# C-bowman/inference-tools

Hardware: AMD Instinct MI355X
Metric: GpRegressor fit+predict wall-time and GFLOP/s at N=16384, d=8; % fp64 MFMA peak (higher is better)
Workload: dtype f64

## Files before the change

inference-tools_amd/csrc/gemm_tiles.h:

```cpp
#pragma once
#include "gpmi_internal.h"

#ifndef GPMI_C_PLAIN
#define GPMI_C_LOAD(p) __builtin_nontemporal_load(p)
#define GPMI_C_STORE(v, p) __builtin_nontemporal_store(v, p)
#else
#define GPMI_C_LOAD(p) (*(p))
#define GPMI_C_STORE(v, p) (*(p) = (v))
#endif

namespace gemm_tiles {

constexpr int CST_NT = 0, CST_SC1 = 1;
template <int CST>
__device__ __forceinline__ void c_store_begin() {
  if (CST == CST_SC1) asm volatile("s_nop 15\n\ts_nop 15" ::: "memory");
}
template <int CST>
__device__ __forceinline__ void c_store(d2_t v, d2_t* p) {
  if (CST == CST_SC1)
    asm volatile("global_store_dwordx4 %0, %1, off sc1\n\ts_nop 1" ::"v"(p), "v"(v) : "memory");
  else
    GPMI_C_STORE(v, p);
}
template <int CST>
__device__ __forceinline__ void c_store(double v, double* p) {
  if (CST == CST_SC1)
    asm volatile("global_store_dwordx2 %0, %1, off sc1" ::"v"(p), "v"(v) : "memory");
  else
    GPMI_C_STORE(v, p);
}

constexpr int BK = 16;
constexpr int LDS_STRIDE = 18;
#ifndef GPMI_SMALL_PF
#define GPMI_SMALL_PF 4
#endif

template <int BKN, int BM, int BN>
constexpr int staged_lds_doubles() {
  return 2 * (BM * LDS_STRIDE + (BKN ? BK * (BN + 16) : BN * LDS_STRIDE));
}

template <int OP, int BKN, int BM, int BN, int CST = CST_NT, bool BTRI = false>
__device__ __forceinline__ void staged_tile(const double* __restrict__ Ag, const double* __restrict__ Bg, double* Cg,
                                            int64_t lda, int64_t ldb, int64_t ldc, int nk, double* smem) {
  static_assert(!BTRI || (BKN == 0 && BN == 128 && OP == OP_ASSIGN), "BTRI: the in-place panel TRSM only");
  constexpr int CSTEP = BTRI ? 32 : 16;
  constexpr int TM = BM / 32, TN = BN / 32;
  constexpr int LDS_STRIDE_KN = BN + 16;
  constexpr int A_DOUBLES = BM * LDS_STRIDE;
  constexpr int B_DOUBLES = BKN ? BK * LDS_STRIDE_KN : BN * LDS_STRIDE;
  constexpr int BUF_DOUBLES = A_DOUBLES + B_DOUBLES;
  const int tid = threadIdx.x;
  const int lane = tid & 63, wave = tid >> 6;
  const int wr = wave >> 1, wc = wave & 1;

  const int lrow = tid >> 3, lkc = (tid & 7) * 2;
  const int lkc_sw = lkc ^ ((((lrow & 15) >= 4) && ((lrow & 15) < 12)) ? 4 : 0);
  const int nrow = tid / (BN / 2), nnc = (tid % (BN / 2)) * 2;
  constexpr int PF = (BM * BN < 128 * 128) ? GPMI_SMALL_PF : 1;
  d2_t ra[PF][TM], rb[PF][TN];
  unsigned voa[TM], vob[TN];
#pragma unroll
  for (int i = 0; i < TM; ++i) voa[i] = (unsigned)(((int64_t)(lrow + 32 * i) * lda + lkc) * 8);
#pragma unroll
  for (int i = 0; i < TN; ++i)
    vob[i] = BKN ? (unsigned)(((int64_t)(nrow + (512 / BN) * i) * ldb + nnc) * 8)
                 : (unsigned)(((int64_t)(lrow + 32 * i) * ldb + lkc) * 8);
  auto gload = [&](int k0, int slot) {
    const char* ab = reinterpret_cast<const char*>(Ag + k0);
    const char* bb = reinterpret_cast<const char*>(BKN ? Bg + (int64_t)k0 * ldb : Bg + k0);
#pragma unroll
    for (int i = 0; i < TM; ++i) ra[slot][i] = *reinterpret_cast<const d2_t*>(ab + voa[i]);
#pragma unroll
    for (int i = 0; i < TN; ++i) rb[slot][i] = *reinterpret_cast<const d2_t*>(bb + vob[i]);
  };
  auto sstore = [&](int buf, int slot) {
    double* sa = smem + buf * BUF_DOUBLES;
    double* sb = sa + A_DOUBLES;
#pragma unroll
    for (int i = 0; i < TM; ++i)
      *reinterpret_cast<d2_t*>(sa + (lrow + 32 * i) * LDS_STRIDE + lkc_sw) = (OP == OP_SUB) ? -ra[slot][i] : ra[slot][i];
#pragma unroll
    for (int i = 0; i < TN; ++i) {
      if (BKN)
        *reinterpret_cast<d2_t*>(sb + (nrow + (512 / BN) * i) * LDS_STRIDE_KN + nnc) = rb[slot][i];
      else
        *reinterpret_cast<d2_t*>(sb + (lrow + 32 * i) * LDS_STRIDE + lkc_sw) = rb[slot][i];
    }
  };

  const int fr = lane & 15, fk = lane >> 4;
  const int wcol = BTRI ? wc * 16 : wc * (BN / 2);
  Cg += (int64_t)(wr * (BM / 2)) * ldc + wcol;
  const int sw = (fr >= 4 && fr < 12) ? 1 : 0;
  const int a_off = (wr * (BM / 2) + fr) * LDS_STRIDE + ((fk ^ sw) << 2);
  const int b_off = BKN ? 4 * fk * LDS_STRIDE_KN + wc * (BN / 2) + fr
                        : (wcol + fr) * LDS_STRIDE + ((fk ^ sw) << 2);

  const int klast = (nk - 1) * BK;
  auto gload_clamped = [&](int kt, int slot) { gload(kt < nk ? kt * BK : klast, slot); };
  if (PF == 1) gload(0, 0);
  d4_t acc[TM][TN];
#pragma unroll
  for (int i = 0; i < TM; ++i)
#pragma unroll
    for (int j = 0; j < TN; ++j) {
      if (OP == OP_SUB) {
#pragma unroll
        for (int r = 0; r < 4; ++r) acc[i][j][r] = GPMI_C_LOAD(&Cg[(int64_t)(i * 16 + fk + 4 * r) * ldc + j * CSTEP + fr]);
      } else {
        acc[i][j] = d4_t{0.0, 0.0, 0.0, 0.0};
      }
    }
  if (PF > 1) {
    gload(0, 0);
#pragma unroll
    for (int p = 1; p < PF; ++p) gload_clamped(p, p);
  }
  sstore(0, 0);
  __syncthreads();
  auto kstep = [&](int kt, int slot_free, int slot_next) {
    const int cur = kt & 1;
    if (PF == 1) {
      if (kt + 1 < nk) gload((kt + 1) * BK, 0);
    } else {
      gload_clamped(kt + PF, slot_free);
    }
    const double* sa = smem + cur * BUF_DOUBLES;
    const double* sb = sa + A_DOUBLES;
#pragma unroll
    for (int h = 0; h < 2; ++h) {
      d2_t a[TM], b[TN];
#pragma unroll
      for (int t = 0; t < TM; ++t)
        a[t] = *reinterpret_cast<const d2_t*>(sa + a_off + t * 16 * LDS_STRIDE + 2 * h);
#pragma unroll
      for (int t = 0; t < TN; ++t) {
        if (BKN)
          b[t] = d2_t{sb[b_off + (2 * h) * LDS_STRIDE_KN + t * 16],
                      sb[b_off + (2 * h + 1) * LDS_STRIDE_KN + t * 16]};
        else
          b[t] = *reinterpret_cast<const d2_t*>(sb + b_off + t * CSTEP * LDS_STRIDE + 2 * h);
      }
#pragma unroll
      for (int j = 0; j < TN; ++j) {
        if (BTRI && kt > 2 * j + wc) continue;
#pragma unroll
        for (int q = 0; q < 2; ++q)
#pragma unroll
          for (int i = 0; i < TM; ++i)
            acc[i][j] = __builtin_amdgcn_mfma_f64_16x16x4f64(a[i][q], b[j][q], acc[i][j], 0, 0, 0);
      }
    }
    if (PF > 1 || kt + 1 < nk) sstore(cur ^ 1, slot_next);
    __syncthreads();
  };
  if (PF == 1) {
    kstep(0, 0, 0);
    for (int kt = 1; kt < nk; ++kt) kstep(kt, 0, 0);
  } else {
    for (int kb = 0; kb < nk; kb += PF) {
#pragma unroll
      for (int u = 0; u < PF; ++u) {
        if (kb + u >= nk) break;
        kstep(kb + u, u, (1 + u) % PF);
      }
    }
  }

  c_store_begin<CST>();
#pragma unroll
  for (int i = 0; i < TM; ++i)
#pragma unroll
    for (int j = 0; j < TN; ++j)
#pragma unroll
      for (int r = 0; r < 4; ++r) c_store<CST>(acc[i][j][r], &Cg[(int64_t)(i * 16 + fk + 4 * r) * ldc + j * CSTEP + fr]);
}

constexpr int DMA_BK = 8;
#ifndef GPMI_DMA_STAGES
#define GPMI_DMA_STAGES 4
#endif
constexpr int DMA_STAGES = GPMI_DMA_STAGES;
constexpr int DMA_OP_DOUBLES = 128 * DMA_BK;
constexpr int DMA128_LDS_DOUBLES = DMA_STAGES * 2 * DMA_OP_DOUBLES;
constexpr int DMA64_LDS_DOUBLES = DMA_STAGES * 2 * 64 * DMA_BK;

__device__ inline void dma_wait(int newer) {
  if (newer >= 12) asm volatile("s_waitcnt vmcnt(12)" ::: "memory");
  else if (newer >= 8) asm volatile("s_waitcnt vmcnt(8)" ::: "memory");
  else if (newer >= 4) asm volatile("s_waitcnt vmcnt(4)" ::: "memory");
  else asm volatile("s_waitcnt vmcnt(0)" ::: "memory");
}

template <int OP, int CST = CST_NT>
__device__ __forceinline__ void dma128_tile(const double* __restrict__ Ag, const double* __restrict__ Bg, double* Cg,
                                            int64_t lda, int64_t ldb, int64_t ldc, int nk, double* smem) {
  const int tid = threadIdx.x, lane = tid & 63, wave = tid >> 6;
  const int wr = wave >> 1, wc = wave & 1;
  const int fr = lane & 15, fk = lane >> 4;
  const int row0 = tid >> 2, slot = tid & 3;
  const int q0 = (slot - 2 * ((row0 >> 2) & 3)) & 3;
  const double* a_src0 = Ag + (int64_t)row0 * lda + 2 * q0;
  const double* a_src1 = a_src0 + (int64_t)64 * lda;
  auto bperm = [](int R) {
    const int t = (R >> 4) & 3, f = R & 15;
    return (R & 64) + ((t & 2) << 4) + 2 * f + (t & 1);
  };
  const double* b_src0 = Bg + (int64_t)bperm(row0) * ldb + 2 * q0;
  const double* b_src1 = Bg + (int64_t)bperm(row0 + 64) * ldb + 2 * q0;
  const unsigned lds0 = (unsigned)(uintptr_t)smem;
  const unsigned wave_off = (unsigned)__builtin_amdgcn_readfirstlane(wave * 64 * 16);
  auto issue = [&](int st, int k0) {
    const unsigned base = lds0 + (unsigned)st * (2 * DMA_OP_DOUBLES * 8) + wave_off;
    const double* p0 = a_src0 + k0;
    const double* p1 = a_src1 + k0;
    const double* p2 = b_src0 + k0;
    const double* p3 = b_src1 + k0;
    asm volatile(
        "s_mov_b32 m0, %4\n\ts_nop 0\n\tglobal_load_lds_dwordx4 %0, off\n\t"
        "s_mov_b32 m0, %5\n\ts_nop 0\n\tglobal_load_lds_dwordx4 %1, off\n\t"
        "s_mov_b32 m0, %6\n\ts_nop 0\n\tglobal_load_lds_dwordx4 %2, off\n\t"
        "s_mov_b32 m0, %7\n\ts_nop 0\n\tglobal_load_lds_dwordx4 %3, off"
        :
        : "v"(p0), "v"(p1), "v"(p2), "v"(p3), "s"(base), "s"(base + 256 * 16), "s"(base + DMA_OP_DOUBLES * 8),
          "s"(base + DMA_OP_DOUBLES * 8 + 256 * 16)
        : "memory");
  };
  for (int st = 0; st < DMA_STAGES - 1 && st < nk; ++st) issue(st, st * DMA_BK);

  Cg += (int64_t)(wr * 64) * ldc + wc * 64;
  d4_t acc[4][4];
#pragma unroll
  for (int i = 0; i < 4; ++i)
#pragma unroll
    for (int jp = 0; jp < 2; ++jp)
#pragma unroll
      for (int r = 0; r < 4; ++r) {
        d2_t cv = d2_t{0.0, 0.0};
        if (OP == OP_SUB)
          cv = GPMI_C_LOAD(reinterpret_cast<const d2_t*>(&Cg[(int64_t)(i * 16 + fk + 4 * r) * ldc + jp * 32 + 2 * fr]));
        acc[i][2 * jp][r] = cv[0];
        acc[i][2 * jp + 1][r] = cv[1];
      }

  const int rslot = (fk + 2 * (fr >> 2)) & 3;
  const int a_off = ((wr * 64 + fr) * 4 + rslot) * 2;
  const int b_off = DMA_OP_DOUBLES + ((wc * 64 + fr) * 4 + rslot) * 2;
  auto stage = [&](int kt) {
    const int ahead = nk - 1 - kt;
    dma_wait(4 * (ahead < DMA_STAGES - 2 ? ahead : DMA_STAGES - 2));
    __syncthreads();
#ifdef GPMI_DMA_ISSUE_EARLY
    if (kt + DMA_STAGES - 1 < nk) issue((kt + DMA_STAGES - 1) % DMA_STAGES, (kt + DMA_STAGES - 1) * DMA_BK);
#endif
    const double* sa = smem + (kt % DMA_STAGES) * 2 * DMA_OP_DOUBLES;
    d2_t a[4], b[4];
#pragma unroll
    for (int t = 0; t < 4; ++t) {
      a[t] = *reinterpret_cast<const d2_t*>(sa + a_off + t * 16 * 4 * 2);
    }
#pragma unroll
    for (int t = 0; t < 4; ++t) b[t] = *reinterpret_cast<const d2_t*>(sa + b_off + t * 16 * 4 * 2);
#ifndef GPMI_DMA_ISSUE_EARLY
    if (kt + DMA_STAGES - 1 < nk) issue((kt + DMA_STAGES - 1) % DMA_STAGES, (kt + DMA_STAGES - 1) * DMA_BK);
#endif
#pragma unroll
    for (int h = 0; h < 2; ++h)
#pragma unroll
      for (int i = 0; i < 4; ++i)
#pragma unroll
        for (int j = 0; j < 4; ++j)
          acc[i][j] = __builtin_amdgcn_mfma_f64_16x16x4f64(a[i][h], b[j][h], acc[i][j], 0, 0, OP == OP_SUB ? 1 : 0);
  };
  stage(0);
  int kt = 1;
  for (; kt + 3 < nk; kt += 4) {
    stage(kt);
    stage(kt + 1);
    stage(kt + 2);
    stage(kt + 3);
  }
  for (; kt < nk; ++kt) stage(kt);
  c_store_begin<CST>();
#pragma unroll
  for (int i = 0; i < 4; ++i)
#pragma unroll
    for (int jp = 0; jp < 2; ++jp)
#pragma unroll
      for (int r = 0; r < 4; ++r)
        c_store<CST>((d2_t{acc[i][2 * jp][r], acc[i][2 * jp + 1][r]}),
                     reinterpret_cast<d2_t*>(&Cg[(int64_t)(i * 16 + fk + 4 * r) * ldc + jp * 32 + 2 * fr]));
}

template <int OP, int CST = CST_NT>
__device__ __forceinline__ void dma64_tile(const double* __restrict__ Ag, const double* __restrict__ Bg, double* Cg,
                                           int64_t lda, int64_t ldb, int64_t ldc, int nk, double* smem) {
  constexpr int OPD = 64 * DMA_BK;
  const int tid = threadIdx.x, lane = tid & 63, wave = tid >> 6;
  const int wr = wave >> 1, wc = wave & 1;
  const int fr = lane & 15, fk = lane >> 4;
  const int row0 = tid >> 2, slot = tid & 3;
  const int q0 = (slot - 2 * ((row0 >> 2) & 3)) & 3;
  const double* a_src = Ag + (int64_t)row0 * lda + 2 * q0;
  const int bcol = (row0 & 32) + 2 * (row0 & 15) + ((row0 >> 4) & 1);
  const double* b_src = Bg + (int64_t)bcol * ldb + 2 * q0;
  const unsigned lds0 = (unsigned)(uintptr_t)smem;
  const unsigned wave_off = (unsigned)__builtin_amdgcn_readfirstlane(wave * 64 * 16);
  auto issue = [&](int st, int k0) {
    const unsigned base = lds0 + (unsigned)st * (2 * OPD * 8) + wave_off;
    const double* p0 = a_src + k0;
    const double* p1 = b_src + k0;
    asm volatile(
        "s_mov_b32 m0, %2\n\ts_nop 0\n\tglobal_load_lds_dwordx4 %0, off\n\t"
        "s_mov_b32 m0, %3\n\ts_nop 0\n\tglobal_load_lds_dwordx4 %1, off"
        :
        : "v"(p0), "v"(p1), "s"(base), "s"(base + OPD * 8)
        : "memory");
  };
  for (int st = 0; st < DMA_STAGES - 1 && st < nk; ++st) issue(st, st * DMA_BK);

  Cg += (int64_t)(wr * 32) * ldc + wc * 32;
  d4_t acc[2][2];
#pragma unroll
  for (int i = 0; i < 2; ++i)
#pragma unroll
    for (int r = 0; r < 4; ++r) {
      d2_t cv = d2_t{0.0, 0.0};
      if (OP == OP_SUB)
        cv = GPMI_C_LOAD(reinterpret_cast<const d2_t*>(&Cg[(int64_t)(i * 16 + fk + 4 * r) * ldc + 2 * fr]));
      acc[i][0][r] = cv[0];
      acc[i][1][r] = cv[1];
    }
  const int rslot = (fk + 2 * (fr >> 2)) & 3;
  const int a_off = ((wr * 32 + fr) * 4 + rslot) * 2;
  const int b_off = OPD + ((wc * 32 + fr) * 4 + rslot) * 2;
  auto wait2 = [](int newer) {
    if (newer >= 6) asm volatile("s_waitcnt vmcnt(6)" ::: "memory");
    else if (newer >= 4) asm volatile("s_waitcnt vmcnt(4)" ::: "memory");
    else if (newer >= 2) asm volatile("s_waitcnt vmcnt(2)" ::: "memory");
    else asm volatile("s_waitcnt vmcnt(0)" ::: "memory");
  };
  auto stage = [&](int kt) {
    const int ahead = nk - 1 - kt;
    wait2(2 * (ahead < DMA_STAGES - 2 ? ahead : DMA_STAGES - 2));
    __syncthreads();
    const double* sa = smem + (kt % DMA_STAGES) * 2 * OPD;
    d2_t a[2], b[2];
#pragma unroll
    for (int t = 0; t < 2; ++t) {
      a[t] = *reinterpret_cast<const d2_t*>(sa + a_off + t * 16 * 4 * 2);
      b[t] = *reinterpret_cast<const d2_t*>(sa + b_off + t * 16 * 4 * 2);
    }
    if (kt + DMA_STAGES - 1 < nk) issue((kt + DMA_STAGES - 1) % DMA_STAGES, (kt + DMA_STAGES - 1) * DMA_BK);
#pragma unroll
    for (int h = 0; h < 2; ++h)
#pragma unroll
      for (int i = 0; i < 2; ++i)
#pragma unroll
        for (int j = 0; j < 2; ++j)
          acc[i][j] = __builtin_amdgcn_mfma_f64_16x16x4f64(a[i][h], b[j][h], acc[i][j], 0, 0, OP == OP_SUB ? 1 : 0);
  };
  stage(0);
  int kt = 1;
  for (; kt + 3 < nk; kt += 4) {
    stage(kt);
    stage(kt + 1);
    stage(kt + 2);
    stage(kt + 3);
  }
  for (; kt < nk; ++kt) stage(kt);
  c_store_begin<CST>();
#pragma unroll
  for (int i = 0; i < 2; ++i)
#pragma unroll
    for (int r = 0; r < 4; ++r)
      c_store<CST>((d2_t{acc[i][0][r], acc[i][1][r]}),
                   reinterpret_cast<d2_t*>(&Cg[(int64_t)(i * 16 + fk + 4 * r) * ldc + 2 * fr]));
}

constexpr int FLOW_SPIN_LIMIT = 1 << 20;

__device__ __forceinline__ int flow_ld(const int* p) {
  return __hip_atomic_load(p, __ATOMIC_RELAXED, __HIP_MEMORY_SCOPE_AGENT);
}

}
```

Measured before the change: 55020.

## Interleave DMA prefetch pieces between MFMAs and use SGPR-base addressing in GEMM tiles

Splits each stage's global-to-LDS prefetch into per-operand pieces and issues them between MFMA instructions, fenced by sched barriers, so the loads hide under matrix math instead of issuing as one burst. Steady-state stages become a compile-time 'full' specialization with a fixed vmcnt wait and no bounds check on the prefetch. Global loads now use a uniform SGPR base plus a 32-bit VGPR offset, which saves VGPRs and address arithmetic. The 32-bit offset could overflow on very large leading dimensions, and the fixed scheduling may interfere with the compiler's own MFMA interleaving.

```diff
diff --git a/inference-tools_amd/csrc/gemm_tiles.h b/inference-tools_amd/csrc/gemm_tiles.h
--- a/inference-tools_amd/csrc/gemm_tiles.h
+++ b/inference-tools_amd/csrc/gemm_tiles.h
@@ -184,6 +184,27 @@
 #define GPMI_DMA_STAGES 4
 #endif
 constexpr int DMA_STAGES = GPMI_DMA_STAGES;
+#ifndef GPMI_RING_SADDR
+#define GPMI_RING_SADDR 1
+#endif
+#ifndef GPMI_RING_STATIC_TRIPS
+#define GPMI_RING_STATIC_TRIPS 1
+#endif
+#ifndef GPMI_RING_DMA_UNDER
+#define GPMI_RING_DMA_UNDER 1
+#endif
+#ifndef GPMI_RING_DMA_FIRST
+#define GPMI_RING_DMA_FIRST 2
+#endif
+#ifndef GPMI_RING_DMA_STEP
+#define GPMI_RING_DMA_STEP 4
+#endif
+#ifndef GPMI_RING_DMA64_FIRST
+#define GPMI_RING_DMA64_FIRST 1
+#endif
+#ifndef GPMI_RING_DMA64_STEP
+#define GPMI_RING_DMA64_STEP 2
+#endif
 constexpr int DMA_OP_DOUBLES = 128 * DMA_BK;
 constexpr int DMA128_LDS_DOUBLES = DMA_STAGES * 2 * DMA_OP_DOUBLES;
 constexpr int DMA64_LDS_DOUBLES = DMA_STAGES * 2 * 64 * DMA_BK;
@@ -195,6 +216,18 @@
   else asm volatile("s_waitcnt vmcnt(0)" ::: "memory");
 }
 
+__device__ __forceinline__ const double* ring_uniform(const double* p) {
+  const unsigned long long v = (unsigned long long)(uintptr_t)p;
+  const unsigned lo = (unsigned)__builtin_amdgcn_readfirstlane((int)(unsigned)v);
+  const unsigned hi = (unsigned)__builtin_amdgcn_readfirstlane((int)(unsigned)(v >> 32));
+  return reinterpret_cast<const double*>((uintptr_t)(((unsigned long long)hi << 32) | lo));
+}
+__device__ __forceinline__ void ring_piece(const double* src, unsigned dst) {
+  asm volatile("s_mov_b32 m0, %1\n\ts_nop 0\n\tglobal_load_lds_dwordx4 %0, off" ::"v"(src), "s"(dst) : "memory");
+}
+__device__ __forceinline__ void ring_piece(unsigned voff, const double* sbase, unsigned dst) {
+  asm volatile("s_mov_b32 m0, %2\n\ts_nop 0\n\tglobal_load_lds_dwordx4 %0, %1" ::"v"(voff), "s"(sbase), "s"(dst) : "memory");
+}
 template <int OP, int CST = CST_NT>
 __device__ __forceinline__ void dma128_tile(const double* __restrict__ Ag, const double* __restrict__ Bg, double* Cg,
                                             int64_t lda, int64_t ldb, int64_t ldc, int nk, double* smem) {
@@ -203,31 +236,31 @@
   const int fr = lane & 15, fk = lane >> 4;
   const int row0 = tid >> 2, slot = tid & 3;
   const int q0 = (slot - 2 * ((row0 >> 2) & 3)) & 3;
-  const double* a_src0 = Ag + (int64_t)row0 * lda + 2 * q0;
-  const double* a_src1 = a_src0 + (int64_t)64 * lda;
   auto bperm = [](int R) {
     const int t = (R >> 4) & 3, f = R & 15;
     return (R & 64) + ((t & 2) << 4) + 2 * f + (t & 1);
   };
-  const double* b_src0 = Bg + (int64_t)bperm(row0) * ldb + 2 * q0;
-  const double* b_src1 = Bg + (int64_t)bperm(row0 + 64) * ldb + 2 * q0;
   const unsigned lds0 = (unsigned)(uintptr_t)smem;
   const unsigned wave_off = (unsigned)__builtin_amdgcn_readfirstlane(wave * 64 * 16);
+  const int64_t src_off[4] = {(int64_t)row0 * lda + 2 * q0, (int64_t)(row0 + 64) * lda + 2 * q0,
+                              (int64_t)bperm(row0) * ldb + 2 * q0, (int64_t)bperm(row0 + 64) * ldb + 2 * q0};
+#if GPMI_RING_SADDR
+  const double* Au = ring_uniform(Ag);
+  const double* Bu = ring_uniform(Bg);
+  const unsigned voff[4] = {(unsigned)(src_off[0] * 8), (unsigned)(src_off[1] * 8), (unsigned)(src_off[2] * 8),
+                            (unsigned)(src_off[3] * 8)};
+#endif
+  auto piece = [&](int p, int st, int k0) {
+    const unsigned dst = lds0 + (unsigned)st * (2 * DMA_OP_DOUBLES * 8) + wave_off + (p >> 1) * (DMA_OP_DOUBLES * 8) + (p & 1) * (256 * 16);
+#if GPMI_RING_SADDR
+    ring_piece(voff[p], (p < 2 ? Au : Bu) + k0, dst);
+#else
+    ring_piece((p < 2 ? Ag : Bg) + src_off[p] + k0, dst);
+#endif
+  };
   auto issue = [&](int st, int k0) {
-    const unsigned base = lds0 + (unsigned)st * (2 * DMA_OP_DOUBLES * 8) + wave_off;
-    const double* p0 = a_src0 + k0;
-    const double* p1 = a_src1 + k0;
-    const double* p2 = b_src0 + k0;
-    const double* p3 = b_src1 + k0;
-    asm volatile(
-        "s_mov_b32 m0, %4\n\ts_nop 0\n\tglobal_load_lds_dwordx4 %0, off\n\t"
-        "s_mov_b32 m0, %5\n\ts_nop 0\n\tglobal_load_lds_dwordx4 %1, off\n\t"
-        "s_mov_b32 m0, %6\n\ts_nop 0\n\tglobal_load_lds_dwordx4 %2, off\n\t"
-        "s_mov_b32 m0, %7\n\ts_nop 0\n\tglobal_load_lds_dwordx4 %3, off"
-        :
-        : "v"(p0), "v"(p1), "v"(p2), "v"(p3), "s"(base), "s"(base + 256 * 16), "s"(base + DMA_OP_DOUBLES * 8),
-          "s"(base + DMA_OP_DOUBLES * 8 + 256 * 16)
-        : "memory");
+#pragma unroll
+    for (int p = 0; p < 4; ++p) piece(p, st, k0);
   };
   for (int st = 0; st < DMA_STAGES - 1 && st < nk; ++st) issue(st, st * DMA_BK);
 
@@ -249,12 +282,16 @@
   const int rslot = (fk + 2 * (fr >> 2)) & 3;
   const int a_off = ((wr * 64 + fr) * 4 + rslot) * 2;
   const int b_off = DMA_OP_DOUBLES + ((wc * 64 + fr) * 4 + rslot) * 2;
-  auto stage = [&](int kt) {
+  auto stage = [&](int kt, auto full) {
+    constexpr bool under = GPMI_RING_DMA_UNDER && decltype(full)::value;
     const int ahead = nk - 1 - kt;
-    dma_wait(4 * (ahead < DMA_STAGES - 2 ? ahead : DMA_STAGES - 2));
+    if (decltype(full)::value) dma_wait(4 * (DMA_STAGES - 2));
+    else dma_wait(4 * (ahead < DMA_STAGES - 2 ? ahead : DMA_STAGES - 2));
     __syncthreads();
+    const bool pf = decltype(full)::value || kt + DMA_STAGES - 1 < nk;
+    const int pf_st = (kt + DMA_STAGES - 1) % DMA_STAGES, pf_k0 = (kt + DMA_STAGES - 1) * DMA_BK;
 #ifdef GPMI_DMA_ISSUE_EARLY
-    if (kt + DMA_STAGES - 1 < nk) issue((kt + DMA_STAGES - 1) % DMA_STAGES, (kt + DMA_STAGES - 1) * DMA_BK);
+    if (!under && pf) issue(pf_st, pf_k0);
 #endif
     const double* sa = smem + (kt % DMA_STAGES) * 2 * DMA_OP_DOUBLES;
     d2_t a[4], b[4];
@@ -265,25 +302,43 @@
 #pragma unroll
     for (int t = 0; t < 4; ++t) b[t] = *reinterpret_cast<const d2_t*>(sa + b_off + t * 16 * 4 * 2);
 #ifndef GPMI_DMA_ISSUE_EARLY
-    if (kt + DMA_STAGES - 1 < nk) issue((kt + DMA_STAGES - 1) % DMA_STAGES, (kt + DMA_STAGES - 1) * DMA_BK);
-#endif
+    if (!under && pf) issue(pf_st, pf_k0);
+#endif
+    int m = 0;
 #pragma unroll
     for (int h = 0; h < 2; ++h)
 #pragma unroll
       for (int i = 0; i < 4; ++i)
 #pragma unroll
-        for (int j = 0; j < 4; ++j)
+        for (int j = 0; j < 4; ++j) {
           acc[i][j] = __builtin_amdgcn_mfma_f64_16x16x4f64(a[i][h], b[j][h], acc[i][j], 0, 0, OP == OP_SUB ? 1 : 0);
-  };
-  stage(0);
+          ++m;
+          if (under && m >= GPMI_RING_DMA_FIRST && (m - GPMI_RING_DMA_FIRST) % GPMI_RING_DMA_STEP == 0 &&
+              (m - GPMI_RING_DMA_FIRST) / GPMI_RING_DMA_STEP < 4) {
+            __builtin_amdgcn_sched_barrier(0);
+            piece((m - GPMI_RING_DMA_FIRST) / GPMI_RING_DMA_STEP, pf_st, pf_k0);
+            __builtin_amdgcn_sched_barrier(0);
+          }
+        }
+  };
+  stage(0, std::false_type{});
   int kt = 1;
+#if GPMI_RING_STATIC_TRIPS || GPMI_RING_DMA_UNDER
+  for (; kt + 3 + DMA_STAGES - 1 < nk; kt += 4) {
+    stage(kt, std::true_type{});
+    stage(kt + 1, std::true_type{});
+    stage(kt + 2, std::true_type{});
+    stage(kt + 3, std::true_type{});
+  }
+#else
   for (; kt + 3 < nk; kt += 4) {
-    stage(kt);
-    stage(kt + 1);
-    stage(kt + 2);
-    stage(kt + 3);
-  }
-  for (; kt < nk; ++kt) stage(kt);
+    stage(kt, std::false_type{});
+    stage(kt + 1, std::false_type{});
+    stage(kt + 2, std::false_type{});
+    stage(kt + 3, std::false_type{});
+  }
+#endif
+  for (; kt < nk; ++kt) stage(kt, std::false_type{});
   c_store_begin<CST>();
 #pragma unroll
   for (int i = 0; i < 4; ++i)
@@ -304,21 +359,26 @@
   const int fr = lane & 15, fk = lane >> 4;
   const int row0 = tid >> 2, slot = tid & 3;
   const int q0 = (slot - 2 * ((row0 >> 2) & 3)) & 3;
-  const double* a_src = Ag + (int64_t)row0 * lda + 2 * q0;
   const int bcol = (row0 & 32) + 2 * (row0 & 15) + ((row0 >> 4) & 1);
-  const double* b_src = Bg + (int64_t)bcol * ldb + 2 * q0;
   const unsigned lds0 = (unsigned)(uintptr_t)smem;
   const unsigned wave_off = (unsigned)__builtin_amdgcn_readfirstlane(wave * 64 * 16);
+  const int64_t src_off[2] = {(int64_t)row0 * lda + 2 * q0, (int64_t)bcol * ldb + 2 * q0};
+#if GPMI_RING_SADDR
+  const double* Au = ring_uniform(Ag);
+  const double* Bu = ring_uniform(Bg);
+  const unsigned voff[2] = {(unsigned)(src_off[0] * 8), (unsigned)(src_off[1] * 8)};
+#endif
+  auto piece = [&](int p, int st, int k0) {
+    const unsigned dst = lds0 + (unsigned)st * (2 * OPD * 8) + wave_off + p * (OPD * 8);
+#if GPMI_RING_SADDR
+    ring_piece(voff[p], (p ? Bu : Au) + k0, dst);
+#else
+    ring_piece((p ? Bg : Ag) + src_off[p] + k0, dst);
+#endif
+  };
   auto issue = [&](int st, int k0) {
-    const unsigned base = lds0 + (unsigned)st * (2 * OPD * 8) + wave_off;
-    const double* p0 = a_src + k0;
-    const double* p1 = b_src + k0;
-    asm volatile(
-        "s_mov_b32 m0, %2\n\ts_nop 0\n\tglobal_load_lds_dwordx4 %0, off\n\t"
-        "s_mov_b32 m0, %3\n\ts_nop 0\n\tglobal_load_lds_dwordx4 %1, off"
-        :
-        : "v"(p0), "v"(p1), "s"(base), "s"(base + OPD * 8)
-        : "memory");
+    piece(0, st, k0);
+    piece(1, st, k0);
   };
   for (int st = 0; st < DMA_STAGES - 1 && st < nk; ++st) issue(st, st * DMA_BK);
 
@@ -343,10 +403,14 @@
     else if (newer >= 2) asm volatile("s_waitcnt vmcnt(2)" ::: "memory");
     else asm volatile("s_waitcnt vmcnt(0)" ::: "memory");
   };
-  auto stage = [&](int kt) {
+  auto stage = [&](int kt, auto full) {
+    constexpr bool under = GPMI_RING_DMA_UNDER && decltype(full)::value;
     const int ahead = nk - 1 - kt;
-    wait2(2 * (ahead < DMA_STAGES - 2 ? ahead : DMA_STAGES - 2));
+    if (decltype(full)::value) wait2(2 * (DMA_STAGES - 2));
+    else wait2(2 * (ahead < DMA_STAGES - 2 ? ahead : DMA_STAGES - 2));
     __syncthreads();
+    const bool pf = decltype(full)::value || kt + DMA_STAGES - 1 < nk;
+    const int pf_st = (kt + DMA_STAGES - 1) % DMA_STAGES, pf_k0 = (kt + DMA_STAGES - 1) * DMA_BK;
     const double* sa = smem + (kt % DMA_STAGES) * 2 * OPD;
     d2_t a[2], b[2];
 #pragma unroll
@@ -354,24 +418,42 @@
       a[t] = *reinterpret_cast<const d2_t*>(sa + a_off + t * 16 * 4 * 2);
       b[t] = *reinterpret_cast<const d2_t*>(sa + b_off + t * 16 * 4 * 2);
     }
-    if (kt + DMA_STAGES - 1 < nk) issue((kt + DMA_STAGES - 1) % DMA_STAGES, (kt + DMA_STAGES - 1) * DMA_BK);
+    if (!under && pf) issue(pf_st, pf_k0);
+    int m = 0;
 #pragma unroll
     for (int h = 0; h < 2; ++h)
 #pragma unroll
       for (int i = 0; i < 2; ++i)
 #pragma unroll
-        for (int j = 0; j < 2; ++j)
+        for (int j = 0; j < 2; ++j) {
           acc[i][j] = __builtin_amdgcn_mfma_f64_16x16x4f64(a[i][h], b[j][h], acc[i][j], 0, 0, OP == OP_SUB ? 1 : 0);
-  };
-  stage(0);
+          ++m;
+          if (under && m >= GPMI_RING_DMA64_FIRST && (m - GPMI_RING_DMA64_FIRST) % GPMI_RING_DMA64_STEP == 0 &&
+              (m - GPMI_RING_DMA64_FIRST) / GPMI_RING_DMA64_STEP < 2) {
+            __builtin_amdgcn_sched_barrier(0);
+            piece((m - GPMI_RING_DMA64_FIRST) / GPMI_RING_DMA64_STEP, pf_st, pf_k0);
+            __builtin_amdgcn_sched_barrier(0);
+          }
+        }
+  };
+  stage(0, std::false_type{});
   int kt = 1;
+#if GPMI_RING_STATIC_TRIPS || GPMI_RING_DMA_UNDER
+  for (; kt + 3 + DMA_STAGES - 1 < nk; kt += 4) {
+    stage(kt, std::true_type{});
+    stage(kt + 1, std::true_type{});
+    stage(kt + 2, std::true_type{});
+    stage(kt + 3, std::true_type{});
+  }
+#else
   for (; kt + 3 < nk; kt += 4) {
-    stage(kt);
-    stage(kt + 1);
-    stage(kt + 2);
-    stage(kt + 3);
-  }
-  for (; kt < nk; ++kt) stage(kt);
+    stage(kt, std::false_type{});
+    stage(kt + 1, std::false_type{});
+    stage(kt + 2, std::false_type{});
+    stage(kt + 3, std::false_type{});
+  }
+#endif
+  for (; kt < nk; ++kt) stage(kt, std::false_type{});
   c_store_begin<CST>();
 #pragma unroll
   for (int i = 0; i < 2; ++i)
```

After: 56740, median of 6. +3.1%, better.
